# hkbharath/MARL-MASS

Hardware: AMD Instinct MI355X
Metric: agent-steps/sec (whole node), MASS CBF shield on, 65536 envs x 8 CAVs (higher is better)
Workload: dtype f64

## Files before the change

### include/mm_math.h

```cpp
#ifndef MM_MATH_H
#define MM_MATH_H

#ifndef MMM_FN
#define MMM_FN static inline
#endif

#if defined(__HIP_DEVICE_COMPILE__) && defined(__gfx950__)
MMM_FN double mmm_fma_c(double p, double z, double c) {
  double r;
  __asm__("v_fma_f64 %0, %1, %2, %3" : "=v"(r) : "v"(p), "v"(z), "s"(c));
  return r;
}
#else
#define mmm_fma_c(p, z, c) fma((p), (z), (c))
#endif

#define MMM_PIO2_1 0x1.921fb54400000p+0
#define MMM_PIO2_1T 0x1.0b4611a626331p-34
#define MMM_PIO2_HI 0x1.921fb54442d18p+0
#define MMM_PIO2_LO 0x1.1a62633145c07p-54
#define MMM_TWO_OVER_PI 0x1.45f306dc9c883p-1
#define MMM_LN2_HI 0x1.62e42ff000000p-1
#define MMM_LN2_LO -0x1.718432a1b0e26p-35
#define MMM_INV_LN2 0x1.71547652b82fep+0
// ... 136 lines not shown
  if (inv) r = MMM_PIO2_HI - (r - MMM_PIO2_LO);
  return x < 0 ? -r : r;
}
MMM_FN double mmm_atan_small(double x) {
  double t = fabs(x);
  double z = t * t;
  double p = MMM_K(mmm_t_atan, 0, MMM_A10);
  p = mmm_fma_c(p, z, MMM_K(mmm_t_atan, 1, MMM_A9)); p = mmm_fma_c(p, z, MMM_K(mmm_t_atan, 2, MMM_A8)); p = mmm_fma_c(p, z, MMM_K(mmm_t_atan, 3, MMM_A7)); p = mmm_fma_c(p, z, MMM_K(mmm_t_atan, 4, MMM_A6));
  p = mmm_fma_c(p, z, MMM_K(mmm_t_atan, 5, MMM_A5)); p = mmm_fma_c(p, z, MMM_K(mmm_t_atan, 6, MMM_A4)); p = mmm_fma_c(p, z, MMM_K(mmm_t_atan, 7, MMM_A3)); p = mmm_fma_c(p, z, MMM_K(mmm_t_atan, 8, MMM_A2));
  p = mmm_fma_c(p, z, MMM_K(mmm_t_atan, 9, MMM_A1));
  double r = fma(t * z, p, t);
  return x < 0 ? -r : r;
}
MMM_FN double mmm_asin_w(double x, double *w_out) {
  double y = fabs(x), lo;
  double w = sqrt((1.0 - y) * (1.0 + y));
  *w_out = w;
  const int direct = y <= w;
  double r = mmm_atan_ratio(direct ? y : w, direct ? w : y, &lo);
  if (!direct) r = MMM_PIO2_HI - (r - MMM_PIO2_LO);
  return x < 0 ? -r : r;
}
MMM_FN double mmm_asin(double x) { double w; return mmm_asin_w(x, &w); }
#define MMM_SIN_PI3 0x1.bb67ae8584caap-1
#define MMM_COS_PI3 0x1.0000000000001p-1
MMM_FN double mmm_exp(double x) {
  if (x < -1000.0) return 0.0;
  double k = rint(x * MMM_INV_LN2);
  double r = fma(-k, MMM_LN2_HI, x);
  r = fma(-k, MMM_LN2_LO, r);
  double p = MMM_K(mmm_t_exp, 0, MMM_E14);
  p = mmm_fma_c(p, r, MMM_K(mmm_t_exp, 1, MMM_E13)); p = mmm_fma_c(p, r, MMM_K(mmm_t_exp, 2, MMM_E12)); p = mmm_fma_c(p, r, MMM_K(mmm_t_exp, 3, MMM_E11)); p = mmm_fma_c(p, r, MMM_K(mmm_t_exp, 4, MMM_E10));
  p = mmm_fma_c(p, r, MMM_K(mmm_t_exp, 5, MMM_E9)); p = mmm_fma_c(p, r, MMM_K(mmm_t_exp, 6, MMM_E8)); p = mmm_fma_c(p, r, MMM_K(mmm_t_exp, 7, MMM_E7)); p = mmm_fma_c(p, r, MMM_K(mmm_t_exp, 8, MMM_E6));
  p = mmm_fma_c(p, r, MMM_K(mmm_t_exp, 9, MMM_E5)); p = mmm_fma_c(p, r, MMM_K(mmm_t_exp, 10, MMM_E4)); p = mmm_fma_c(p, r, MMM_K(mmm_t_exp, 11, MMM_E3)); p = mmm_fma_c(p, r, MMM_K(mmm_t_exp, 12, MMM_E2));
  p = fma(p, r * r, r) + 1.0;
  return ldexp(p, (int)k);
}
MMM_FN double mmm_log(double x) {
  int e;
  double m = frexp(x, &e);
  if (m < MMM_SQRT_HALF) { m = m * 2.0; e -= 1; }
  double f = m - 1.0;
  double s = f / (2.0 + f);
  double z = s * s;
  double p = MMM_K(mmm_t_log, 0, MMM_L11);
  p = mmm_fma_c(p, z, MMM_K(mmm_t_log, 1, MMM_L10)); p = mmm_fma_c(p, z, MMM_K(mmm_t_log, 2, MMM_L9)); p = mmm_fma_c(p, z, MMM_K(mmm_t_log, 3, MMM_L8)); p = mmm_fma_c(p, z, MMM_K(mmm_t_log, 4, MMM_L7));
// ... 19 lines not shown
```

### marl-mass_amd/csrc/mm_device.h

```cpp
#pragma once
#include <hip/hip_runtime.h>
#include <stdint.h>

#include "../../include/mm_abi.h"

#define MM_DEV __device__ __forceinline__
#define MMM_FN __device__ __forceinline__
#include "../../include/mm_math.h"
#ifndef MM_QP_NO_CERTIFY
#define MM_QP_CERTIFY
#endif
#include "../../include/mm_qp.h"

namespace mm {

constexpr double kPi = 3.141592653589793;
constexpr double kVehLength = 5.0, kVehWidth = 2.0, kMaxSpeed = 40.0;
constexpr double kTauA = 0.6, kTauDs = 0.2;
constexpr double kLcMaxAcc = 6.0, kLcMinAcc = -12.5;
constexpr double kPerception = 180.0, kStoppingSpeed = 1.6667;
constexpr double kLaneWidth = 4.0;
constexpr double kCbfAccLo = -12.5, kCbfAccHi = 6.0, kAdjBuffer = 2.0134;
constexpr double kSineAmp = 3.25, kSinePuls = 2 * kPi / (2 * 100.0), kSinePhase = kPi / 2;
constexpr double kObstX = 420.0, kObstY = 4.0;
constexpr double kT180 = 0x1.fa3ffffffffffp+14;
constexpr double kU5 = 0x1.9000000000001p+4;
constexpr double kCornerLen = 2.7000824035672517;
constexpr double kCornerAlpha = 0.3805063771123649;

MM_DEV double lane_sx(int l) { return l == 0 ? 0.0 : (l <= 2 ? 320.0 : (l == 3 ? 420.0 : (l == 4 ? 0.0 : 220.0))); }
MM_DEV double lane_sy(int l) { return l == 2 ? 4.0 : (l == 4 ? 10.5 : (l == 5 ? 7.25 : 0.0)); }
MM_DEV double lane_len(int l) { return l == 0 ? 320.0 : (l == 3 ? 1000.0 : (l == 4 ? 220.0 : 100.0)); }
MM_DEV bool lane_forbidden(int l) { return l == 2 || l >= 4; }
MM_DEV int lane_road(int l) { return l == 0 ? 0 : (l <= 2 ? 1 : l - 1); }
MM_DEV int lane_rid(int l) { return l == MM_LANE_BC1 ? 1 : 0; }

MM_DEV double fmod_pos(double a, double b) {
// ... 13 lines not shown
  if (m != 0.0) {
    if (m < 0) m += b;
  } else {
    m = 0.0;
  }
  return m;
}
MM_DEV double wrap_to_pi(double x) {
  const double a = x + kPi;
  if (__all(a >= 0.0 && a < 2 * kPi)) return a - kPi;
  return py_mod(a, 2 * kPi) - kPi;
}
MM_DEV double not_zero(double x) {
  return fabs(x) > 1e-2 ? x : (x > 0 ? 1e-2 : -1e-2);
}
MM_DEV double clipd(double x, double a, double b) { return fmin(fmax(x, a), b); }
MM_DEV double div_c(double x, double d, double y) {
  const double q = x * y;
  const double r = fma(-q, d, x);
  return fma(r, y, q);
}
#define MM_DIVC(x, d) ::mm::div_c((x), (d), 1.0 / (d))

MM_DEV void lane_local(int l, double x, double y, double &s, double &r) {
  s = x - lane_sx(l);
  r = y - lane_sy(l);
  if (l == MM_LANE_KB0) r = r - kSineAmp * mmm_sin(kSinePuls * s + kSinePhase);
}
MM_DEV void lane_local_carried(int l, double x, double y, double car, double &s, double &r) {
  s = x - lane_sx(l);
  r = y - lane_sy(l);
  const bool kb = l == MM_LANE_KB0;
  double sn = car;
  if (__any(kb && car != car)) sn = (car != car) ? mmm_sin(kSinePuls * s + kSinePhase) : car;
  if (kb) r = r - kSineAmp * sn;
}
static_assert(kSineAmp * kSinePuls * (1.0 + 0x1p-40) < 0.125, "the sine lane's heading needs the general mmm_atan");
template <bool SINE = false>
MM_DEV double lane_heading_at(int l, double s) {
  if constexpr (SINE) return l == MM_LANE_KB0 ? 0.0 + mmm_atan_small(kSineAmp * kSinePuls * mmm_cos(kSinePuls * s + kSinePhase)) : 0.0;
  else return l == MM_LANE_KB0 ? 0.0 + mmm_atan(kSineAmp * kSinePuls * mmm_cos(kSinePuls * s + kSinePhase)) : 0.0;
}
MM_DEV double lane_distance(int l, double x, double y) {
  double s, r;
  lane_local(l, x, y, s, r);
  return fabs(r) + fmax(s - lane_len(l), 0.0) + fmax(0.0 - s, 0.0);
}
MM_DEV bool lane_on_lane(int l, double x, double y) {
  double s, r;
  lane_local(l, x, y, s, r);
  return fabs(r) <= kLaneWidth / 2 + 0 && (-kVehLength <= s && s < lane_len(l) + kVehLength);
}
MM_DEV bool lane_reachable(int l, double x, double y) {
  if (lane_forbidden(l)) return false;
  double s = x - lane_sx(l), r = y - lane_sy(l);
  return fabs(r) <= 2 * kLaneWidth && (0 <= s && s < lane_len(l) + kVehLength);
}
MM_DEV bool lane_after_end(int l, double x) {
  return (x - lane_sx(l)) > lane_len(l) - kVehLength / 2;
}

template <bool SINE = false>
MM_DEV int closest_lane(double x, double y, double h, double *sine_out = nullptr) {
// ... 25 lines not shown
      double d = fabs(r) + tail + head + 1.0 * fabs(wrap_to_pi(h - lh));
      if (d < bd) { bd = d; best = MM_LANE_KB0; }
    }
  }
  return best;
}
MM_DEV int next_lane(int l, double x, double y) {
  if (l == MM_LANE_AB0 || l == MM_LANE_KB0)
    return lane_distance(MM_LANE_BC0, x, y) <= lane_distance(MM_LANE_BC1, x, y) ? MM_LANE_BC0 : MM_LANE_BC1;
  if (l == MM_LANE_JK0) return MM_LANE_KB0;
  return MM_LANE_CD0;
}

MM_DEV int speed_to_index(double speed) {
  double x = MM_DIVC(speed - 10, 20.0);
  return (int)clipd(rint(x * (5 - 1)), 0, 5 - 1);
}
MM_DEV double index_to_speed(int i) { return 10 + i * (30.0 - 10) / (5 - 1); }

template <bool SINE = false, bool CARRIED = false>
MM_DEV double steering_control(double x, double y, double heading, double speed, int tl, double &half_tan, double car = 0.0) {
  constexpr double KP_HEADING = 1 / kTauDs, KP_LATERAL = 1.0 / 3 * KP_HEADING, PURSUIT_TAU = 0.5 * kTauDs;
  double s, r;
  if constexpr (CARRIED) lane_local_carried(tl, x, y, car, s, r);
  else lane_local(tl, x, y, s, r);
  double lane_next = s + speed * PURSUIT_TAU;
  double lfh = lane_heading_at<SINE>(tl, lane_next);
  double lat_cmd = -KP_LATERAL * r;
  double nz = not_zero(speed);
  double heading_command = mmm_asin(clipd(lat_cmd / nz, -1, 1));
  double heading_ref = lfh + clipd(heading_command, -kPi / 4, kPi / 4);
  double rate = KP_HEADING * wrap_to_pi(heading_ref - heading);
  const double arg = clipd(kVehLength / 2 / nz * rate, -1, 1);
  double w;
  const double steer = mmm_asin_w(arg, &w);
  const bool sat = fabs(steer) > kPi / 3;
  const double ss = sat ? (arg < 0 ? -MMM_SIN_PI3 : MMM_SIN_PI3) : arg;
  const double cs = sat ? MMM_COS_PI3 : w;
  half_tan = 1.0 / 2 * (ss / cs);
  return clipd(steer, -kPi / 3, kPi / 3);
}
MM_DEV double steering_control(double x, double y, double heading, double speed, int tl) {
  double ht;
  return steering_control(x, y, heading, speed, tl, ht);
}

MM_DEV bool has_corner_inside(double c1x, double c1y, double l1, double w1, double a1, double c2x,
                              double c2y, double l2, double w2, double a2) {
  const double lx = l1 / 2, wy = w1 / 2;
  double c = mmm_cos(a1), s = mmm_sin(a1), c2 = mmm_cos(a2), s2 = mmm_sin(a2);
  const double px[9] = {0, -lx, lx, 0, 0, -lx, -lx, lx, lx};
  const double py[9] = {0, 0, 0, -wy, wy, -wy, wy, -wy, wy};
  bool any = false;
#pragma unroll
  for (int k = 0; k < 9; k++) {
    double rx = c * px[k] + (-s) * py[k], ry = s * px[k] + c * py[k];
    double dx = (c1x + rx) - c2x, dy = (c1y + ry) - c2y;
    double ru0 = c2 * dx + (-s2) * dy, ru1 = s2 * dx + c2 * dy;
// ... 37 lines not shown
```

### marl-mass_amd/csrc/mm_kernels.hip

```cpp
#include <hip/hip_runtime.h>
#include <math.h>
#include <stdio.h>
#include <string.h>

#include <type_traits>

#include "mm_device.h"
#include "mm_div.h"
#include "mm_handle.h"
#define MM_COUNTS_FN __host__ __device__ inline
#include "../../include/mm_counts.h"
#include "../../include/mm_policy_wide.h"

using namespace mm;

struct DevCfg {
  int env_kind, shield, nsub, T, action_masking, auto_reset, obs_f64, N, E, debug_flags, n_hdv;
  double dt, collision_reward, high_speed_reward, headway_cost, headway_time, merging_lane_cost;
  double rs_lo, rs_hi, eta, tau;
  double inv_dt, rs_span, rs_ispan, rs_span2, rs_ispan2;
  int agent_reward;
  int steer_vel;
  int *err;
  int traffic_density, mixed_traffic, num_cav;
// ... 60 lines not shown
    unsigned long long _t = __builtin_amdgcn_s_memtime();                                \
    if ((threadIdx.x & 63) == (k)) _t_acc += _t - _t_last;                               \
    _t_last = __builtin_amdgcn_s_memtime();                                              \
  } while (0)
enum { MM_CS_UPFRONT_CYCLES = 16,
       MM_CS_UPFRONT,
       MM_CS_LAZY_B,
       MM_CS_FALLBACK,
       MM_CS_PRIOR_HELD,
       MM_CS_PRIOR_LIFTED,
       MM_CS_LAZY_A,
       MM_CS_FIRST_B,
       MM_CS_NEAR,
       MM_CS_NEAR_ANY,
       MM_CS_PRECHECK,
       MM_CS_ROUND_CYCLES,
       MM_CS_ROUNDS,
       MM_CS_PASSES,
       MM_CS_SEED_ACTIVE,
       MM_CS_DIAG_CYCLES };
static_assert(MM_CS_DIAG_CYCLES == 31, "sixteen slots: lanes 16 .. 31");
constexpr bool mm_cs_is_cycles(int slot) { return slot == MM_CS_UPFRONT_CYCLES || slot == MM_CS_ROUND_CYCLES || slot == MM_CS_DIAG_CYCLES; }
__device__ unsigned long long g_stamps_c[MM_STAMP_WAVES * 16];
#define CAND_COUNT(k, cond)                                                                                  \
  do {                                                                                                       \
    const unsigned long long _m = __ballot(cond);                                                            \
    if ((threadIdx.x & 63) == (k)) _t_acc += (unsigned long long)__popcll(_m) + (_m ? 1ull << 32 : 0ull);    \
  } while (0)
#else
#define STAMP(k) do {} while (0)
#define SSTAMP(k) do {} while (0)
#define SCOUNT(k) do {} while (0)
#define CAND_COUNT(k, cond) do {} while (0)
#endif

template <int KIND> constexpr bool kIdm = KIND == MM_ENV_HDV_V1;

struct Veh {
  double x, y, h, v, tspeed;
  double act_steer, act_acc, safe_steer, safe_acc, gvx;
  double h1x, h1vx, h2x, h2vx;
  double sang;
  int lane, tlane, sidx, crashed, hl, flags, hist_len;
  int kind;
  bool present;
};
// ... 30 lines not shown
template <int M, int G, class F>
MM_DEV void for_partners_impl(F &f) {
  if constexpr (M < G) {
    f(std::integral_constant<int, M>{});
    for_partners_impl<M + 1, G>(f);
  }
}
template <int G, class F>
MM_DEV void for_partners(F f) { for_partners_impl<1, G>(f); }

template <int G> constexpr bool kPow2 = (G & (G - 1)) == 0;
#ifndef MM_ROUNDS_LITE
#define MM_ROUNDS_LITE 1
#endif
constexpr bool kRoundsLite = MM_ROUNDS_LITE != 0;
#ifndef MM_ROUNDS_PRIOR
#define MM_ROUNDS_PRIOR 1
#endif
constexpr bool kRoundsPrior = MM_ROUNDS_PRIOR != 0;
#ifndef MM_SCAN_SELECTS
#define MM_SCAN_SELECTS 1
#endif
constexpr bool kScanSelects = MM_SCAN_SELECTS != 0;
#ifndef MM_VETO_PRIOR
#define MM_VETO_PRIOR 1
#endif
constexpr bool kVetoPrior = MM_VETO_PRIOR != 0;
template <int M, int G>
MM_DEV int pidx(int a) {
  if constexpr (kPow2<G>) return a ^ M;
  else return a + M >= G ? a + M - G : a + M;
}
template <int G>
MM_DEV int pidx_rt(int a, int m) {
  if constexpr (kPow2<G>) return a ^ m;
  else return a + m >= G ? a + m - G : a + m;
}
template <int M, int G>
MM_DEV int plane(int lane, int a) {
  if constexpr (kPow2<G>) return lane ^ M;
  else return lane - a + pidx<M, G>(a);
}
template <int G>
MM_DEV int plane_rt(int lane, int a, int m) {
  if constexpr (kPow2<G>) return lane ^ m;
  else return lane - a + pidx_rt<G>(a, m);
// ... 90 lines not shown
    int cand = v.tlane;
    if (lane_road(v.tlane) == 1) cand = (action == 2) ? MM_LANE_BC1 : MM_LANE_BC0;
    if (lane_reachable(cand, v.x, v.y)) v.tlane = cand;
  }
  v.act_acc = (1 / kTauA) * (v.tspeed - v.v);
  if constexpr (STEER) steer_lane<SINE>(v, sv, st_t);
}
template <int KIND>
MM_DEV void hl_act(Veh &v, int action) {
  if (KIND == MM_ENV_V1 && action >= 0) v.hl = action;
  if (action == 3 || action == 4) {
    int si = speed_to_index(v.v) + (action == 3 ? 1 : -1);
    v.sidx = si < 0 ? 0 : (si > 4 ? 4 : si);
    v.tspeed = index_to_speed(v.sidx);
  }
  if (lane_after_end(v.tlane, v.x)) v.tlane = next_lane(v.tlane, v.x, v.y);
  if (action == 2 || action == 0) {
    int cand = v.tlane;
    if (lane_road(v.tlane) == 1) cand = (action == 2) ? MM_LANE_BC1 : MM_LANE_BC0;
    if (lane_reachable(cand, v.x, v.y)) v.tlane = cand;
  }
}

MM_DEV void clip_actions(Veh &v, bool lc_vehicle, double &st_t) {
  if (v.crashed) { v.act_steer = 0; st_t = 0; v.act_acc = -1.0 * v.v; }
  if (v.v > kMaxSpeed) v.act_acc = fmin(v.act_acc, 1.0 * (kMaxSpeed - v.v));
  else if (v.v < -kMaxSpeed) v.act_acc = fmax(v.act_acc, 1.0 * (kMaxSpeed - v.v));
  if (lc_vehicle) v.act_acc = clipd(v.act_acc, kLcMinAcc, kLcMaxAcc);
}

MM_DEV int corner_flags(double x, double y, double sh, double ch, int lane) {
  double cx = x + (kCornerLen * mmm_cos_sum(MMM_CORNER_SIN, MMM_CORNER_COS, sh, ch));
  double cyL = y - (kCornerLen * mmm_sin_sum(MMM_CORNER_SIN, MMM_CORNER_COS, sh, ch)) + 0.01;
  double cyR = y - (kCornerLen * mmm_sin_sum(-MMM_CORNER_SIN, MMM_CORNER_COS, sh, ch)) + 0.01;
  double s = cx - lane_sx(lane);
  double off = (lane == MM_LANE_KB0) ? kSineAmp * mmm_sin(kSinePuls * s + kSinePhase) : 0.0;
  bool lon = (-kVehLength <= s && s < lane_len(lane) + kVehLength);
  double rL = cyL - lane_sy(lane), rR = cyR - lane_sy(lane);
  if (lane == MM_LANE_KB0) { rL = rL - off; rR = rR - off; }
  return (!(fabs(rL) <= kLaneWidth / 2 + 0 && lon) ? 1 : 0) | (!(fabs(rR) <= kLaneWidth / 2 + 0 && lon) ? 2 : 0);
}
MM_DEV int pose_code(int lane, int nl, int off) { return lane | nl << 3 | off << 6; }

struct Cand {
  double x, y, h, gvx, cpsi, spsi;
  int lane;
  int pk;
};
template <int KIND, bool SHIELDED, bool CORNERS = SHIELDED, bool GENERAL = true, bool SINE = false>
MM_DEV Cand predict(const Veh &v, double steer, double st_t, double sh, double ch, double dt, bool sv = false, double *sine_out = nullptr) {
  Cand c;
  double ht = st_t, sb, cb;
  if constexpr (GENERAL) {
    if (__any(sv || st_t != st_t)) {
      double s2, c2;
      mmm_sincos(sv ? v.sang : steer, &s2, &c2);
      if (sv || st_t != st_t) ht = 1.0 / 2 * (s2 / c2);
    }
  }
  mmm_slip_sincos(ht, &sb, &cb);
  double vx = v.v * mmm_cos_sum(sh, ch, sb, cb), vy = v.v * mmm_sin_sum(sh, ch, sb, cb);
  c.x = v.x + vx * dt;
  c.y = v.y + vy * dt;
  const double d_heading = MM_DIVC(v.v * sb, 2.5);
  c.h = v.h + (sv ? d_heading : d_heading * dt);
  mmm_sincos(c.h, &c.spsi, &c.cpsi);
  c.gvx = (KIND == MM_ENV_V1) ? mmm_cos_sum(c.spsi, c.cpsi, sb, cb) : 0.0;
  c.lane = closest_lane<SINE>(c.x, c.y, c.h, sine_out);
  c.pk = c.lane;
  if (SHIELDED) c.pk = pose_code(c.lane, next_lane(c.lane, c.x, c.y), CORNERS ? corner_flags(c.x, c.y, c.spsi, c.cpsi, c.lane) : 0);
  return c;
}

MM_DEV int adj_pair(int l1, int l2) {
  return (l1 == MM_LANE_BC0 && l2 == MM_LANE_BC1) ? -1 : ((l1 == MM_LANE_BC1 && l2 == MM_LANE_BC0) ? 1 : 0);
}
MM_DEV int adj_lane(int l1, int nl1, int l2) {
  const int f = adj_pair(l1, l2);
  return f != 0 ? f : adj_pair(nl1, l2);
}
MM_DEV unsigned adj_row(int l1) { return l1 == MM_LANE_BC0 ? (3u << (2 * MM_LANE_BC1)) : (l1 == MM_LANE_BC1 ? (1u << (2 * MM_LANE_BC0)) : 0u); }
MM_DEV unsigned adj_col(int l2) { return l2 == MM_LANE_BC1 ? (3u << (2 * MM_LANE_BC0)) : (l2 == MM_LANE_BC0 ? (1u << (2 * MM_LANE_BC1)) : 0u); }

struct QpTrace {
  double rows, a, h0, h1, h2, h3, d, margin;
};

MM_DEV void init_vehicle(Veh &v) {
  v.lane = closest_lane(v.x, v.y, v.h);
  v.tlane = v.lane;
  v.act_steer = v.act_acc = 0;
  v.safe_steer = v.safe_acc = 0;
  if (v.kind == 2) {
// ... 884 lines not shown
#ifdef MM_SERIAL_ALL
  constexpr bool kSerialOnly = true || IPM;
#else
#ifdef MM_SERIAL_MASS
  constexpr bool kSerialOnly = MIXED || MASS || IPM;
#else
  constexpr bool kSerialOnly = MIXED;
#endif
#endif
  constexpr bool kSine = SHIELDED && !SPLIT && !MIXED && !IPM && !kSerialOnly && kPow2<G> && G <= 8;
  constexpr bool kScan = kScanSelects && !MIXED && !TRACE;
#ifndef MM_CARRY_POSE
#define MM_CARRY_POSE 1
#endif
  constexpr bool kCarry = kSine && MM_CARRY_POSE != 0;
#ifndef MM_PRIMARY_PRIOR
#define MM_PRIMARY_PRIOR 1
#endif
  constexpr bool kPrimary = kSine && !TRACE && kVetoPrior && MM_PRIMARY_PRIOR != 0;
#ifndef MM_SINE_CARRY
#define MM_SINE_CARRY 0
#endif
  constexpr bool kSineCarry = kPrimary && MM_SINE_CARRY != 0;
  double car_sn = __builtin_nan("");
  (void)car_sn;
  static_assert(kPow2<G> || MM_STEP_BLOCK == 64, "rotation layouts: one wave per workgroup");
  const long long gtid = (long long)blockIdx.x * blockDim.x + threadIdx.x;
  constexpr int kTail = kPow2<G> ? 64 : (64 / G) * G;
  const bool tail = lane_id() >= kTail;
  const int gb = kPow2<G> ? (lane_id() & ~(G - 1)) : (tail ? kTail - G : lane_id() - lane_id() % G);
  const int a = kPow2<G> ? (int)(gtid % G) : lane_id() - gb;
  const long long e = kPow2<G> ? gtid / G : (tail ? (long long)st.E : (gtid >> 6) * (64 / G) + lane_id() / G);
  const bool valid = e < st.E && a < st.N;
  const long long i = e * st.N + a;
  const long long A = st.A;
  const double dt = c.dt;

#ifdef MM_STAMPS
  unsigned long long _t_last = __builtin_amdgcn_s_memtime(), _t_acc = 0;
#endif
  Veh v;
  const bool sv = MIXED && KIND == MM_ENV_V1 && c.steer_vel != 0;
  int steps = 0, time = 0, n_merge = 0, episode = 0;
  int car_code = 0;
  long long car_kx = 0, car_ky = 0, car_kh = 0;
  double car_s = 0.0, car_c = 1.0;
  if constexpr (kCarry) {
    if (valid) {
      car_kx = __double_as_longlong(pb.F[PB_KX * A + i]); car_ky = __double_as_longlong(pb.F[PB_KY * A + i]);
      car_kh = __double_as_longlong(pb.F[PB_KH * A + i]);
      car_s = pb.F[PB_SIN * A + i]; car_c = pb.F[PB_COS * A + i]; car_code = pb.code[i];
    }
  }
  load_veh(st, i, valid, v, sv);
  if (e < st.E) {
    steps = st.I[MM_E_STEPS * st.E + e]; time = st.I[MM_E_TIME * st.E + e];
  }
  if (!MIXED && v.kind == 2) v.kind = 1;
  if (IDM && v.present) v.kind = 2;
  const bool hdv = MIXED && v.kind == 2;
  const bool ctrl = IDM ? v.present : (v.present && !hdv);
  const bool ctrl_x = IDM ? false : ctrl;
  int action = (!IDM && valid && ctrl) ? actions[i] : 1;
  if ((unsigned)action > 4u) {
    if (!SPLIT || kb == 0) atomicOr(c.err, MM_LATCH_BAD_ACTION);
    action = 1;
  }
  const unsigned present_bits = group_ballot<G>(v.present, gb);
  const unsigned ctrl_bits = group_ballot<G>(ctrl, gb);
  const int n_veh = __popc(present_bits), n_ctrl = __popc(ctrl_bits);
  if (!SPLIT || kb == 0) steps += 1;

  double cpsi = 1.0, spsi = 0.0;
  double st_t = __builtin_nan("");
  int pk_self = v.lane;
  bool carried = false;
  if constexpr (kCarry) {
    const bool hit = car_kx == __double_as_longlong(v.x) && car_ky == __double_as_longlong(v.y) && car_kh == __double_as_longlong(v.h) &&
                     (car_code >> 8) == ((kPoseWritten >> 8) | (MASS ? 1 : 0)) && (car_code & 7) == v.lane;
    carried = !__any(v.present && !hit);
    if (carried && v.present) { spsi = car_s; cpsi = car_c; pk_self = car_code & 0xFF; }
  }
  if (!carried) {
    if (v.present) mmm_sincos(v.h, &spsi, &cpsi);
    if (SHIELDED && v.present) pk_self = pose_code(v.lane, next_lane(v.lane, v.x, v.y), MASS ? corner_flags(v.x, v.y, spsi, cpsi, v.lane) : 0);
  }

  enum { C_B = 0, C_H1X = 8, C_H1VX, C_H2X, C_H2VX, C_SSTEER, C_SACC, C_TSPEED, C_A = 15, C_GU0 = 23, C_GU1 = 24, C_PRE = 25, C_MSGW = 29 };
  constexpr bool kMailbox = G <= 8 || !kPow2<G>;
  constexpr bool kPackMsg = !kPow2<G>;
  constexpr int kColdB = kMailbox ? (kPackMsg ? 29 : 30) : 25;
  constexpr bool kRoomy = false;
  constexpr int C_CPSI = kColdB + G - 1, C_GVX = C_CPSI + 1;
  constexpr int kColdN = !SHIELDED ? 15 : (kSerialOnly ? 23 : kColdB + G - 1 + (kRoomy ? 2 : 0));
  static_assert(kColdN * MM_STEP_BLOCK * 8 >= (MM_STEP_BLOCK / 64) * 64 * 30 * 4, "the obs staging must fit in the cold slots");
  __shared__ double s_cold[kColdN][MM_STEP_BLOCK];
  const int tid = threadIdx.x;
  auto cold_i = [&](int slot, int col) -> int & { return ((int *)&s_cold[slot][col])[0]; };
  if (LC) {
    s_cold[C_H1X][tid] = v.h1x; s_cold[C_H1VX][tid] = v.h1vx; s_cold[C_H2X][tid] = v.h2x; s_cold[C_H2VX][tid] = v.h2vx;
    s_cold[C_SSTEER][tid] = v.safe_steer; s_cold[C_SACC][tid] = v.safe_acc;
  }
  s_cold[C_TSPEED][tid] = v.tspeed;
  if constexpr (kRoomy) { s_cold[C_CPSI][tid] = cpsi; s_cold[C_GVX][tid] = v.gvx; }
  auto CPSI = [&]() -> double { if constexpr (kRoomy) return s_cold[C_CPSI][tid]; else return cpsi; };
  auto GVX = [&]() -> double { if constexpr (kRoomy) return s_cold[C_GVX][tid]; else return v.gvx; };
  bool env_active = IDM ? n_veh > 0 : n_ctrl > 0;
  if constexpr (SPLIT) {
    if (kb > 0) env_active = e < st.E && sb.envf[e] != 0;
  }
  STAMP(0);
  const int k_lo = SPLIT ? (kb > 0 ? kb - 1 : 0) : 0, k_hi = SPLIT ? (kb < c.nsub ? kb : c.nsub - 1) : c.nsub - 1;
  for (int k = k_lo; k <= k_hi; k++) {
    const bool head = !SPLIT || k == kb, tail = !SPLIT || k != kb;
    const bool live = env_active && v.present;
    QpTrace qt = {0, __builtin_nan(""), __builtin_nan(""), __builtin_nan(""), __builtin_nan(""),
                  __builtin_nan(""), __builtin_nan(""), __builtin_nan("")};
    int rank = 0;
    if ((SHIELDED || MIXED) && head) {
      for_partners<G>([&](auto mc) {
        constexpr int m = decltype(mc)::value;
        double px = px_d<m, G>(v.x, a);
        bool pp = px_i<m, G>((int)live, a) != 0;
        if constexpr (kScan) rank += (pp & ((px > v.x) | ((px == v.x) & (pidx<m, G>(a) < a)))) ? 1 : 0;
        else rank += (pp && (px > v.x || (px == v.x && pidx<m, G>(a) < a))) ? 1 : 0;
      });
// ... 88 lines not shown
          const int nxt = (acting && lc_branch) ? ((same_road && hit) ? v.lane : my_tl) : tl_post;
          const bool changed = nxt != tl_post;
          tl_post = nxt;
          if (!__any(changed)) break;
        }
        if constexpr (MIXED) { STAMP(5); }
        if (acting) {
          v.tlane = tl_post;
          v.act_acc = clipd(acc_f0, -6.0, 6.0);
        }
      }
      if (head && live && (!hdv || !v.crashed)) steer_lane(v, sv && !hdv, st_t);
      if (head && hdv && live) v.gvx += dt;
    }
    bool first_B = false;
    if constexpr (kPrimary) {
      static_assert(!MIXED && !SPLIT, "kPrimary: no HDVs, no steer_vel, every launch a whole step");
      first_B = (c.debug_flags & 1) == 0 && live && v.hist_len >= 2 && (v.tlane != v.lane || v.crashed) && !(v.flags & MM_FLAG_IS_LC_SAFE);
      if (live) {
        const int tl_1 = v.tlane + (first_B ? v.lane - v.tlane : 0);
        const double steer = steering_control<kSine, kSineCarry>(v.x, v.y, v.h, v.v, tl_1, st_t, car_sn);
        v.act_steer = clipd(steer, -kPi / 3, kPi / 3);
        const double steer_1 = v.act_steer, st_t_1 = st_t;
        clip_actions(v, LC, st_t);
        if (first_B) { v.act_steer = steer_1; st_t = st_t_1; }
      }
    } else {
      if (live && head) clip_actions(v, LC && !hdv, st_t);
    }
    STAMP(1);
    Cand cA;
    memset(&cA, 0, sizeof cA);
    const bool shield_on = SHIELDED && live && !hdv && v.hist_len >= 2;
    if constexpr (kSineCarry) car_sn = __builtin_nan("");
    if (live && head) cA = predict<KIND, SHIELDED, MASS, MIXED, kSine>(v, v.act_steer, st_t, spsi, cpsi, dt, sv && !hdv, kSineCarry ? &car_sn : nullptr);
    auto park = [&](auto base_c, const Cand &cc, double steer) {
      constexpr int base = decltype(base_c)::value;
      if constexpr (SHIELDED) {
        s_cold[base + 0][tid] = cc.x; s_cold[base + 1][tid] = cc.y; s_cold[base + 2][tid] = cc.h;
        cold_i(base + 3, tid) = cc.pk; s_cold[base + 4][tid] = cc.cpsi; s_cold[base + 5][tid] = steer;
        s_cold[base + 6][tid] = cc.gvx; s_cold[base + 7][tid] = cc.spsi;
      }
    };
    auto park_at = [&](int base, const Cand &cc, double steer) {
      s_cold[base + 0][tid] = cc.x; s_cold[base + 1][tid] = cc.y; s_cold[base + 2][tid] = cc.h;
      cold_i(base + 3, tid) = cc.pk; s_cold[base + 4][tid] = cc.cpsi; s_cold[base + 5][tid] = steer;
      s_cold[base + 6][tid] = cc.gvx; s_cold[base + 7][tid] = cc.spsi;
    };
    if constexpr (kPrimary) park_at(first_B ? (int)C_B : (int)C_A, cA, v.act_steer);
    else if (head) park(std::integral_constant<int, C_A>{}, cA, v.act_steer);
    STAMP(2);
// ... 712 lines not shown
    if (is_mdp(i_rr)) { sum += r_rr; cnt++; }
    regional = sum / cnt;
  }
  double rsum = 0, ssum = 0, tsum = 0;
#pragma unroll
  for (int q = 0; q < G; q++) {
    const double lr = shfl_d(local, gb + q), sp = shfl_d(v.v, gb + q);
    const bool in = q < st.N, cq = in & (((ctrl_bits >> q) & 1u) != 0), pq = in & (((present_bits >> q) & 1u) != 0);
    const double r1 = rsum + lr, s1 = ssum + sp, t1 = tsum + sp;
    rsum = cq ? r1 : rsum; ssum = cq ? s1 : ssum;
    tsum = pq ? t1 : tsum;
  }
  const double reward = env_ok ? rsum / n_ctrl : 0, avg_speed = env_ok ? ssum / n_ctrl : 0;
  const double traffic_speed = env_ok ? tsum / n_veh : 0;
  double th = INFINITY;
  if (ctrl) {
    double h2d = hd;
    if (fabs(kObstY - v.y) <= 2 && kObstX > v.x) { double dd = kObstX - v.x; if (dd < h2d) h2d = dd; }
    h2d = h2d - kVehLength;
    double vx = v.v * cpsi;
    th = h2d / (vx > 1 ? vx : 1);
  }
  const double min_headway = group_min_d<G>(th, a);
  if (e < st.E) { n_merge = st.I[MM_E_N_MERGE * st.E + e]; episode = st.I[MM_E_EPISODE * st.E + e]; }
  double merge_pct = __builtin_nan("");
  if (done) {
    const int n_rem = __popc(group_ballot<G>(
        ctrl && (v.lane == MM_LANE_BC1 || v.lane == MM_LANE_KB0 || v.lane == MM_LANE_JK0), gb));
    merge_pct = n_merge > 0 ? (double)(n_merge - n_rem) / n_merge * 100 : 100.0;
  }
  if (valid) {
    if (out.agents_rewards) out.agents_rewards[i] = ctrl ? local : 0;
    if (out.regional_rewards) out.regional_rewards[i] = ctrl ? regional : 0;
    if (out.agents_dones) out.agents_dones[i] = ctrl ? (uint8_t)(v.crashed || steps >= c.T || v.x < 0) : 1;
    if (out.crashed) out.crashed[i] = v.present ? (uint8_t)v.crashed : 0;
    if (out.agents_info) {
      out.agents_info[i * 3 + 0] = v.present ? v.x : 0;
      out.agents_info[i * 3 + 1] = v.present ? v.y : 0;
      out.agents_info[i * 3 + 2] = v.present ? v.v : 0;
    }
  }
  if (e < st.E && a == 0 && env_ok) {
    if (out.reward) out.reward[e] = reward;
    if (out.done) out.done[e] = (uint8_t)done;
    if (out.average_speed) out.average_speed[e] = avg_speed;
    if (out.traffic_speed) out.traffic_speed[e] = traffic_speed;
    if (out.min_headway) out.min_headway[e] = min_headway;
// ... 39 lines not shown
    memset(&nv, 0, sizeof nv);
    int nm = 0;
    int nc = n_ctrl, nh = n_veh - n_ctrl;
    if constexpr (IDM) { nc = 0; nh = n_veh; }
    episode_counts<KIND>(c, seed, (uint32_t)episode, nc, nh);
    const bool spawn = valid && (c.traffic_density > 0 ? a < nc + nh : v.present);
    if (spawn) nm = spawn_vehicle(nv, a, nc, nh, seed, (uint32_t)episode);
    if (c.traffic_density > 0 && valid) {
      if (!spawn) {
        if (v.present) {
          Veh z;
          memset(&z, 0, sizeof z);
          store_veh(st, i, z, true);
        }
        v.present = false; v.kind = 0;
      }
      st.B[MM_B_KIND * A + i] = spawn ? (uint8_t)nv.kind : (uint8_t)0;
    }
    if (spawn) {
      v = nv;
      spsi = 0.0; cpsi = 1.0;
      if constexpr (kCarry) {
        mmm_sincos(v.h, &car_s, &car_c);
        pk_self = pose_code(v.lane, next_lane(v.lane, v.x, v.y), MASS ? corner_flags(v.x, v.y, car_s, car_c, v.lane) : 0);
      }
      s_cold[C_H1X][tid] = v.h1x; s_cold[C_H1VX][tid] = v.h1vx; s_cold[C_H2X][tid] = v.h2x; s_cold[C_H2VX][tid] = v.h2vx;
      s_cold[C_SSTEER][tid] = v.safe_steer; s_cold[C_SACC][tid] = v.safe_acc; s_cold[C_TSPEED][tid] = v.tspeed;
    }
    n_merge = shfl_i(nm, gb);
    steps = 0; time = 0; episode += 1;
  }
  if (valid && v.present) {
    if (LC) {
      v.h1x = s_cold[C_H1X][tid]; v.h1vx = s_cold[C_H1VX][tid]; v.h2x = s_cold[C_H2X][tid]; v.h2vx = s_cold[C_H2VX][tid];
      if (!hdv) { v.safe_steer = s_cold[C_SSTEER][tid]; v.safe_acc = s_cold[C_SACC][tid]; }
    }
    v.tspeed = s_cold[C_TSPEED][tid];
    store_veh(st, i, v, sv);
    if constexpr (kCarry) {
      pb.F[PB_KX * A + i] = v.x; pb.F[PB_KY * A + i] = v.y; pb.F[PB_KH * A + i] = v.h;
      pb.F[PB_SIN * A + i] = car_s; pb.F[PB_COS * A + i] = car_c;
      pb.code[i] = (pk_self & 0xFF) | (MASS ? 0x100 : 0) | kPoseWritten;
    }
  }
  if (e < st.E && a == 0) {
    st.I[MM_E_STEPS * st.E + e] = steps; st.I[MM_E_TIME * st.E + e] = time;
    st.I[MM_E_N_MERGE * st.E + e] = n_merge; st.I[MM_E_EPISODE * st.E + e] = episode;
  }
  STAMP(11);
  __syncthreads();
  STAMP(14);
  const double sc_h[2] = {spsi, cpsi};
  observe<G, KIND, true, kScan>(c, v, a, gb, i, valid, out.obs, out.action_mask, (float *)&s_cold[0][0], sc_h);
  STAMP(12);
#ifdef MM_STAMPS
  {
    const long long wv = gtid >> 6;
    if ((threadIdx.x & 63) < 16 && wv < MM_STAMP_WAVES) g_stamps_w[wv * 16 + (threadIdx.x & 63)] += _t_acc;
    else if ((threadIdx.x & 63) < 32 && wv < MM_STAMP_WAVES) g_stamps_c[wv * 16 + (threadIdx.x & 63) - 16] += _t_acc;
  }
#endif
}

template <int G, int KIND>
__global__ __launch_bounds__(256) void reset_kernel(DevCfg c, DevState st, int mode, const uint8_t *env_mask,
                                                    const uint64_t *seeds_in, void *obs, uint8_t *avail) {
  const long long gtid = (long long)blockIdx.x * blockDim.x + threadIdx.x;
  const long long e = gtid / G;
  const int a = (int)(gtid % G);
  const int gb = lane_id() & ~(G - 1);
  const bool valid = e < st.E && a < st.N;
  const long long i = e * st.N + a;
  const bool selected = e < st.E && mode != 2 && (!env_mask || env_mask[e]);
  Veh v;
  load_veh(st, i, valid, v);
  if (kIdm<KIND> && v.present) v.kind = 2;
  if (selected) {
    int steps = 0, time = 0, n_merge = 0, episode = st.I[MM_E_EPISODE * st.E + e];
    if (mode == 0) {
      if (seeds_in && a == 0) st.seeds[e] = seeds_in[e];
      const uint64_t seed = seeds_in ? seeds_in[e] : st.seeds[e];
      int nm = 0;
// ... 1125 lines not shown
  hipError_t rc = hipMemcpyFromSymbol(host, HIP_SYMBOL(g_stamps_s), sizeof host);
  for (int k = 0; k < 8; k++) out8[k] = 0;
  for (int w = 0; w < 4096; w++)
    for (int k = 0; k < 8; k++) out8[k] += host[w * 8 + k];
  if (rc == hipSuccess && reset) {
    memset(host, 0, sizeof host);
    rc = hipMemcpyToSymbol(HIP_SYMBOL(g_stamps_s), host, sizeof host);
  }
  return rc == hipSuccess ? MM_OK : MM_ERR_DEVICE;
}
extern "C" int32_t mm_debug_read_stamps(unsigned long long *out16, int32_t reset) {
  static unsigned long long *host = nullptr;
  if (!host) host = (unsigned long long *)malloc(sizeof(unsigned long long) * MM_STAMP_WAVES * 16);
  hipError_t rc = hipMemcpyFromSymbol(host, HIP_SYMBOL(g_stamps_w), sizeof(unsigned long long) * MM_STAMP_WAVES * 16);
  for (int k = 0; k < 16; k++) out16[k] = 0;
  for (long long w = 0; w < MM_STAMP_WAVES; w++)
    for (int k = 0; k < 16; k++) out16[k] += host[w * 16 + k];
  if (rc == hipSuccess && reset) {
    memset(host, 0, sizeof(unsigned long long) * MM_STAMP_WAVES * 16);
    rc = hipMemcpyToSymbol(HIP_SYMBOL(g_stamps_w), host, sizeof(unsigned long long) * MM_STAMP_WAVES * 16);
  }
  return rc == hipSuccess ? MM_OK : MM_ERR_DEVICE;
}
extern "C" int32_t mm_debug_read_cand_stamps(unsigned long long *out32, int32_t reset) {
  static unsigned long long *host = nullptr;
  if (!host) host = (unsigned long long *)malloc(sizeof(unsigned long long) * MM_STAMP_WAVES * 16);
  hipError_t rc = hipMemcpyFromSymbol(host, HIP_SYMBOL(g_stamps_c), sizeof(unsigned long long) * MM_STAMP_WAVES * 16);
  for (int k = 0; k < 32; k++) out32[k] = 0;
  for (long long w = 0; w < MM_STAMP_WAVES; w++)
    for (int k = 0; k < 16; k++) {
      const unsigned long long x = host[w * 16 + k];
      if (mm_cs_is_cycles(k + 16)) { out32[k] += x; continue; }
      out32[k] += x & 0xFFFFFFFFull;
      out32[16 + k] += x >> 32;
    }
  if (rc == hipSuccess && reset) {
    memset(host, 0, sizeof(unsigned long long) * MM_STAMP_WAVES * 16);
    rc = hipMemcpyToSymbol(HIP_SYMBOL(g_stamps_c), host, sizeof(unsigned long long) * MM_STAMP_WAVES * 16);
  }
  return rc == hipSuccess ? MM_OK : MM_ERR_DEVICE;
}
#endif
#endif
```

Baseline: 2.534 billion.

## Use branch-free select variants for trig, asin, corner flags and action clipping; hoist loads

Adds select-based sin/cos, atan-ratio and asin variants that compute both kernels and pick the result instead of branching. It also makes corner_flags and clip_actions branch-free on the sine path, and moves the action and per-env episode counter loads to the top of the step kernel. The counters are stashed in the free high words of shared slots. The goal is less wave divergence and earlier memory latency, paid for with extra ALU work per lane and some shared-memory aliasing. Per-wave timing records are added under the stamps debug build only.

After: 2.595 billion (median of 6 runs). +2.4%, better.

```diff
diff --git a/include/mm_math.h b/include/mm_math.h
--- a/include/mm_math.h
+++ b/include/mm_math.h
@@ -182,6 +182,49 @@
   return x < 0 ? -r : r;
 }
 MMM_FN double mmm_asin(double x) { double w; return mmm_asin_w(x, &w); }
+
+MMM_FN double mmm_sin_sel(double x) {
+  int q;
+  double r = mmm_reduce(x, &q);
+  double ks = mmm_ksin(r), kc = mmm_kcos(r);
+  double s = (q & 1) ? kc : ks;
+  return (q & 2) ? -s : s;
+}
+MMM_FN double mmm_cos_sel(double x) {
+  int q;
+  double r = mmm_reduce(x, &q);
+  double ks = mmm_ksin(r), kc = mmm_kcos(r);
+  double c = (q & 1) ? ks : kc;
+  return ((q + 1) & 2) ? -c : c;
+}
+MMM_FN double mmm_atan_ratio_sel(double num, double den, double *lo_out) {
+  const int j = (num >= 0.125 * den) + (num >= 0.375 * den) + (num >= 0.625 * den) + (num >= 0.875 * den);
+  double c = 0.25 * (double)j;
+  double t = (num - c * den) / (den + c * num);
+  double z = t * t;
+  double p = MMM_K(mmm_t_atan, 0, MMM_A10);
+  p = mmm_fma_c(p, z, MMM_K(mmm_t_atan, 1, MMM_A9)); p = mmm_fma_c(p, z, MMM_K(mmm_t_atan, 2, MMM_A8)); p = mmm_fma_c(p, z, MMM_K(mmm_t_atan, 3, MMM_A7)); p = mmm_fma_c(p, z, MMM_K(mmm_t_atan, 4, MMM_A6));
+  p = mmm_fma_c(p, z, MMM_K(mmm_t_atan, 5, MMM_A5)); p = mmm_fma_c(p, z, MMM_K(mmm_t_atan, 6, MMM_A4)); p = mmm_fma_c(p, z, MMM_K(mmm_t_atan, 7, MMM_A3)); p = mmm_fma_c(p, z, MMM_K(mmm_t_atan, 8, MMM_A2));
+  p = mmm_fma_c(p, z, MMM_K(mmm_t_atan, 9, MMM_A1));
+  double pt = fma(t * z, p, t);
+  double hi = 0.0, lo = 0.0;
+  hi = j >= 1 ? MMM_ATAN_HI_1 : hi; lo = j >= 1 ? MMM_ATAN_LO_1 : lo;
+  hi = j >= 2 ? MMM_ATAN_HI_2 : hi; lo = j >= 2 ? MMM_ATAN_LO_2 : lo;
+  hi = j >= 3 ? MMM_ATAN_HI_3 : hi; lo = j >= 3 ? MMM_ATAN_LO_3 : lo;
+  hi = j >= 4 ? MMM_ATAN_HI_4 : hi; lo = j >= 4 ? MMM_ATAN_LO_4 : lo;
+  *lo_out = lo;
+  return hi + (pt + lo);
+}
+MMM_FN double mmm_asin_w_sel(double x, double *w_out) {
+  double y = fabs(x), lo;
+  double w = sqrt((1.0 - y) * (1.0 + y));
+  *w_out = w;
+  const int direct = y <= w;
+  double r = mmm_atan_ratio_sel(direct ? y : w, direct ? w : y, &lo);
+  if (!direct) r = MMM_PIO2_HI - (r - MMM_PIO2_LO);
+  return x < 0 ? -r : r;
+}
+MMM_FN double mmm_asin_sel(double x) { double w; return mmm_asin_w_sel(x, &w); }
 #define MMM_SIN_PI3 0x1.bb67ae8584caap-1
 #define MMM_COS_PI3 0x1.0000000000001p-1
 MMM_FN double mmm_exp(double x) {
diff --git a/marl-mass_amd/csrc/mm_device.h b/marl-mass_amd/csrc/mm_device.h
--- a/marl-mass_amd/csrc/mm_device.h
+++ b/marl-mass_amd/csrc/mm_device.h
@@ -13,6 +13,25 @@
 #include "../../include/mm_qp.h"
 
 namespace mm {
+
+#ifndef MM_TRIG_SELECTS
+#define MM_TRIG_SELECTS 1
+#endif
+#ifndef MM_ATAN_SELECTS
+#define MM_ATAN_SELECTS 1
+#endif
+#ifndef MM_CORNER_SELECTS
+#define MM_CORNER_SELECTS 1
+#endif
+#ifndef MM_CLIP_SELECTS
+#define MM_CLIP_SELECTS 1
+#endif
+constexpr bool kTrigSelects = MM_TRIG_SELECTS != 0, kAtanSelects = MM_ATAN_SELECTS != 0;
+constexpr bool kCornerSelects = MM_CORNER_SELECTS != 0, kClipSelects = MM_CLIP_SELECTS != 0;
+template <bool SEL> MM_DEV double sin_f(double x) { if constexpr (SEL && kTrigSelects) return mmm_sin_sel(x); else return mmm_sin(x); }
+template <bool SEL> MM_DEV double cos_f(double x) { if constexpr (SEL && kTrigSelects) return mmm_cos_sel(x); else return mmm_cos(x); }
+template <bool SEL> MM_DEV double asin_f(double x) { if constexpr (SEL && kAtanSelects) return mmm_asin_sel(x); else return mmm_asin(x); }
+template <bool SEL> MM_DEV double asin_w_f(double x, double *w) { if constexpr (SEL && kAtanSelects) return mmm_asin_w_sel(x, w); else return mmm_asin_w(x, w); }
 
 constexpr double kPi = 3.141592653589793;
 constexpr double kVehLength = 5.0, kVehWidth = 2.0, kMaxSpeed = 40.0;
@@ -72,23 +91,25 @@
 }
 #define MM_DIVC(x, d) ::mm::div_c((x), (d), 1.0 / (d))
 
+template <bool SEL = false>
 MM_DEV void lane_local(int l, double x, double y, double &s, double &r) {
   s = x - lane_sx(l);
   r = y - lane_sy(l);
-  if (l == MM_LANE_KB0) r = r - kSineAmp * mmm_sin(kSinePuls * s + kSinePhase);
-}
+  if (l == MM_LANE_KB0) r = r - kSineAmp * sin_f<SEL>(kSinePuls * s + kSinePhase);
+}
+template <bool SEL = false>
 MM_DEV void lane_local_carried(int l, double x, double y, double car, double &s, double &r) {
   s = x - lane_sx(l);
   r = y - lane_sy(l);
   const bool kb = l == MM_LANE_KB0;
   double sn = car;
-  if (__any(kb && car != car)) sn = (car != car) ? mmm_sin(kSinePuls * s + kSinePhase) : car;
+  if (__any(kb && car != car)) sn = (car != car) ? sin_f<SEL>(kSinePuls * s + kSinePhase) : car;
   if (kb) r = r - kSineAmp * sn;
 }
 static_assert(kSineAmp * kSinePuls * (1.0 + 0x1p-40) < 0.125, "the sine lane's heading needs the general mmm_atan");
 template <bool SINE = false>
 MM_DEV double lane_heading_at(int l, double s) {
-  if constexpr (SINE) return l == MM_LANE_KB0 ? 0.0 + mmm_atan_small(kSineAmp * kSinePuls * mmm_cos(kSinePuls * s + kSinePhase)) : 0.0;
+  if constexpr (SINE) return l == MM_LANE_KB0 ? 0.0 + mmm_atan_small(kSineAmp * kSinePuls * cos_f<true>(kSinePuls * s + kSinePhase)) : 0.0;
   else return l == MM_LANE_KB0 ? 0.0 + mmm_atan(kSineAmp * kSinePuls * mmm_cos(kSinePuls * s + kSinePhase)) : 0.0;
 }
 MM_DEV double lane_distance(int l, double x, double y) {
@@ -160,18 +181,18 @@
 MM_DEV double steering_control(double x, double y, double heading, double speed, int tl, double &half_tan, double car = 0.0) {
   constexpr double KP_HEADING = 1 / kTauDs, KP_LATERAL = 1.0 / 3 * KP_HEADING, PURSUIT_TAU = 0.5 * kTauDs;
   double s, r;
-  if constexpr (CARRIED) lane_local_carried(tl, x, y, car, s, r);
-  else lane_local(tl, x, y, s, r);
+  if constexpr (CARRIED) lane_local_carried<SINE>(tl, x, y, car, s, r);
+  else lane_local<SINE>(tl, x, y, s, r);
   double lane_next = s + speed * PURSUIT_TAU;
   double lfh = lane_heading_at<SINE>(tl, lane_next);
   double lat_cmd = -KP_LATERAL * r;
   double nz = not_zero(speed);
-  double heading_command = mmm_asin(clipd(lat_cmd / nz, -1, 1));
+  double heading_command = asin_f<SINE>(clipd(lat_cmd / nz, -1, 1));
   double heading_ref = lfh + clipd(heading_command, -kPi / 4, kPi / 4);
   double rate = KP_HEADING * wrap_to_pi(heading_ref - heading);
   const double arg = clipd(kVehLength / 2 / nz * rate, -1, 1);
   double w;
-  const double steer = mmm_asin_w(arg, &w);
+  const double steer = asin_w_f<SINE>(arg, &w);
   const bool sat = fabs(steer) > kPi / 3;
   const double ss = sat ? (arg < 0 ? -MMM_SIN_PI3 : MMM_SIN_PI3) : arg;
   const double cs = sat ? MMM_COS_PI3 : w;
diff --git a/marl-mass_amd/csrc/mm_kernels.hip b/marl-mass_amd/csrc/mm_kernels.hip
--- a/marl-mass_amd/csrc/mm_kernels.hip
+++ b/marl-mass_amd/csrc/mm_kernels.hip
@@ -106,6 +106,9 @@
 static_assert(MM_CS_DIAG_CYCLES == 31, "sixteen slots: lanes 16 .. 31");
 constexpr bool mm_cs_is_cycles(int slot) { return slot == MM_CS_UPFRONT_CYCLES || slot == MM_CS_ROUND_CYCLES || slot == MM_CS_DIAG_CYCLES; }
 __device__ unsigned long long g_stamps_c[MM_STAMP_WAVES * 16];
+#define MM_REC_WAVES (1 << 14)
+enum { MM_REC_BEGIN, MM_REC_END, MM_REC_RT_BEGIN, MM_REC_RT_END, MM_REC_HW, MM_REC_RESPAWN, MM_REC_SLOTS = 8, MM_REC_WORDS = 40 };
+__device__ unsigned long long g_wave_rec[MM_REC_WAVES * MM_REC_WORDS];
 #define CAND_COUNT(k, cond)                                                                                  \
   do {                                                                                                       \
     const unsigned long long _m = __ballot(cond);                                                            \
@@ -182,6 +185,9 @@
 #define MM_SCAN_SELECTS 1
 #endif
 constexpr bool kScanSelects = MM_SCAN_SELECTS != 0;
+#ifndef MM_EARLY_LOADS
+#define MM_EARLY_LOADS 1
+#endif
 #ifndef MM_VETO_PRIOR
 #define MM_VETO_PRIOR 1
 #endif
@@ -318,19 +324,43 @@
   }
 }
 
+template <bool SEL = false>
 MM_DEV void clip_actions(Veh &v, bool lc_vehicle, double &st_t) {
+  if constexpr (SEL && kClipSelects) {
+    const bool cr = v.crashed != 0;
+    v.act_steer = cr ? 0.0 : v.act_steer; st_t = cr ? 0.0 : st_t;
+    double acc = cr ? -1.0 * v.v : v.act_acc;
+    const double room = 1.0 * (kMaxSpeed - v.v);
+    const bool over = v.v > kMaxSpeed, under = !over & (v.v < -kMaxSpeed);
+    const double a_lo = fmin(acc, room), a_hi = fmax(acc, room);
+    acc = over ? a_lo : (under ? a_hi : acc);
+    const double a_lc = clipd(acc, kLcMinAcc, kLcMaxAcc);
+    v.act_acc = lc_vehicle ? a_lc : acc;
+  } else {
   if (v.crashed) { v.act_steer = 0; st_t = 0; v.act_acc = -1.0 * v.v; }
   if (v.v > kMaxSpeed) v.act_acc = fmin(v.act_acc, 1.0 * (kMaxSpeed - v.v));
   else if (v.v < -kMaxSpeed) v.act_acc = fmax(v.act_acc, 1.0 * (kMaxSpeed - v.v));
   if (lc_vehicle) v.act_acc = clipd(v.act_acc, kLcMinAcc, kLcMaxAcc);
-}
-
+  }
+}
+
+template <bool SEL = false>
 MM_DEV int corner_flags(double x, double y, double sh, double ch, int lane) {
   double cx = x + (kCornerLen * mmm_cos_sum(MMM_CORNER_SIN, MMM_CORNER_COS, sh, ch));
   double cyL = y - (kCornerLen * mmm_sin_sum(MMM_CORNER_SIN, MMM_CORNER_COS, sh, ch)) + 0.01;
   double cyR = y - (kCornerLen * mmm_sin_sum(-MMM_CORNER_SIN, MMM_CORNER_COS, sh, ch)) + 0.01;
   double s = cx - lane_sx(lane);
-  double off = (lane == MM_LANE_KB0) ? kSineAmp * mmm_sin(kSinePuls * s + kSinePhase) : 0.0;
+  if constexpr (SEL && kCornerSelects) {
+    const bool kb = lane == MM_LANE_KB0;
+    double sn = 0.0;
+    if (kb) sn = sin_f<true>(kSinePuls * s + kSinePhase);
+    const double off = kb ? kSineAmp * sn : 0.0;
+    const bool lon = (-kVehLength <= s) & (s < lane_len(lane) + kVehLength);
+    const double rL0 = cyL - lane_sy(lane), rR0 = cyR - lane_sy(lane);
+    const double rL = kb ? rL0 - off : rL0, rR = kb ? rR0 - off : rR0;
+    return (!((fabs(rL) <= kLaneWidth / 2 + 0) & lon) ? 1 : 0) | (!((fabs(rR) <= kLaneWidth / 2 + 0) & lon) ? 2 : 0);
+  }
+  double off = (lane == MM_LANE_KB0) ? kSineAmp * sin_f<SEL>(kSinePuls * s + kSinePhase) : 0.0;
   bool lon = (-kVehLength <= s && s < lane_len(lane) + kVehLength);
   double rL = cyL - lane_sy(lane), rR = cyR - lane_sy(lane);
   if (lane == MM_LANE_KB0) { rL = rL - off; rR = rR - off; }
@@ -364,7 +394,7 @@
   c.gvx = (KIND == MM_ENV_V1) ? mmm_cos_sum(c.spsi, c.cpsi, sb, cb) : 0.0;
   c.lane = closest_lane<SINE>(c.x, c.y, c.h, sine_out);
   c.pk = c.lane;
-  if (SHIELDED) c.pk = pose_code(c.lane, next_lane(c.lane, c.x, c.y), CORNERS ? corner_flags(c.x, c.y, c.spsi, c.cpsi, c.lane) : 0);
+  if (SHIELDED) c.pk = pose_code(c.lane, next_lane(c.lane, c.x, c.y), CORNERS ? corner_flags<SINE>(c.x, c.y, c.spsi, c.cpsi, c.lane) : 0);
   return c;
 }
 
@@ -1295,6 +1325,7 @@
 #define MM_SINE_CARRY 0
 #endif
   constexpr bool kSineCarry = kPrimary && MM_SINE_CARRY != 0;
+  constexpr bool kEarly = kSine && MM_EARLY_LOADS != 0;
   double car_sn = __builtin_nan("");
   (void)car_sn;
   static_assert(kPow2<G> || MM_STEP_BLOCK == 64, "rotation layouts: one wave per workgroup");
@@ -1310,6 +1341,7 @@
   const double dt = c.dt;
 
 #ifdef MM_STAMPS
+  const unsigned long long _rec_t0 = __builtin_amdgcn_s_memtime(), _rec_rt0 = __builtin_amdgcn_s_memrealtime();
   unsigned long long _t_last = __builtin_amdgcn_s_memtime(), _t_acc = 0;
 #endif
   Veh v;
@@ -1318,6 +1350,12 @@
   int car_code = 0;
   long long car_kx = 0, car_ky = 0, car_kh = 0;
   double car_s = 0.0, car_c = 1.0;
+  int act_raw = 1;
+  (void)act_raw;
+  if constexpr (kEarly) {
+    if (valid) act_raw = actions[i];
+    if (e < st.E) { n_merge = st.I[MM_E_N_MERGE * st.E + e]; episode = st.I[MM_E_EPISODE * st.E + e]; }
+  }
   if constexpr (kCarry) {
     if (valid) {
       car_kx = __double_as_longlong(pb.F[PB_KX * A + i]); car_ky = __double_as_longlong(pb.F[PB_KY * A + i]);
@@ -1334,7 +1372,9 @@
   const bool hdv = MIXED && v.kind == 2;
   const bool ctrl = IDM ? v.present : (v.present && !hdv);
   const bool ctrl_x = IDM ? false : ctrl;
-  int action = (!IDM && valid && ctrl) ? actions[i] : 1;
+  int action;
+  if constexpr (kEarly) action = ctrl ? act_raw : 1;
+  else action = (!IDM && valid && ctrl) ? actions[i] : 1;
   if ((unsigned)action > 4u) {
     if (!SPLIT || kb == 0) atomicOr(c.err, MM_LATCH_BAD_ACTION);
     action = 1;
@@ -1356,7 +1396,7 @@
   }
   if (!carried) {
     if (v.present) mmm_sincos(v.h, &spsi, &cpsi);
-    if (SHIELDED && v.present) pk_self = pose_code(v.lane, next_lane(v.lane, v.x, v.y), MASS ? corner_flags(v.x, v.y, spsi, cpsi, v.lane) : 0);
+    if (SHIELDED && v.present) pk_self = pose_code(v.lane, next_lane(v.lane, v.x, v.y), MASS ? corner_flags<kSine>(v.x, v.y, spsi, cpsi, v.lane) : 0);
   }
 
   enum { C_B = 0, C_H1X = 8, C_H1VX, C_H2X, C_H2VX, C_SSTEER, C_SACC, C_TSPEED, C_A = 15, C_GU0 = 23, C_GU1 = 24, C_PRE = 25, C_MSGW = 29 };
@@ -1375,6 +1415,10 @@
     s_cold[C_SSTEER][tid] = v.safe_steer; s_cold[C_SACC][tid] = v.safe_acc;
   }
   s_cold[C_TSPEED][tid] = v.tspeed;
+  if constexpr (kEarly) {
+    static_assert(kMailbox && !kPackMsg, "the high words of the pose-code and rank-word slots must be free");
+    ((int *)&s_cold[C_PRE + 3][tid])[1] = n_merge; ((int *)&s_cold[C_MSGW][tid])[1] = episode;
+  }
   if constexpr (kRoomy) { s_cold[C_CPSI][tid] = cpsi; s_cold[C_GVX][tid] = v.gvx; }
   auto CPSI = [&]() -> double { if constexpr (kRoomy) return s_cold[C_CPSI][tid]; else return cpsi; };
   auto GVX = [&]() -> double { if constexpr (kRoomy) return s_cold[C_GVX][tid]; else return v.gvx; };
@@ -1509,11 +1553,11 @@
         const double steer = steering_control<kSine, kSineCarry>(v.x, v.y, v.h, v.v, tl_1, st_t, car_sn);
         v.act_steer = clipd(steer, -kPi / 3, kPi / 3);
         const double steer_1 = v.act_steer, st_t_1 = st_t;
-        clip_actions(v, LC, st_t);
+        clip_actions<kSine>(v, LC, st_t);
         if (first_B) { v.act_steer = steer_1; st_t = st_t_1; }
       }
     } else {
-      if (live && head) clip_actions(v, LC && !hdv, st_t);
+      if (live && head) clip_actions<kSine>(v, LC && !hdv, st_t);
     }
     STAMP(1);
     Cand cA;
@@ -2272,7 +2316,8 @@
     th = h2d / (vx > 1 ? vx : 1);
   }
   const double min_headway = group_min_d<G>(th, a);
-  if (e < st.E) { n_merge = st.I[MM_E_N_MERGE * st.E + e]; episode = st.I[MM_E_EPISODE * st.E + e]; }
+  if constexpr (kEarly) { n_merge = ((const int *)&s_cold[C_PRE + 3][tid])[1]; episode = ((const int *)&s_cold[C_MSGW][tid])[1]; }
+  else if (e < st.E) { n_merge = st.I[MM_E_N_MERGE * st.E + e]; episode = st.I[MM_E_EPISODE * st.E + e]; }
   double merge_pct = __builtin_nan("");
   if (done) {
     const int n_rem = __popc(group_ballot<G>(
@@ -2358,7 +2403,7 @@
       spsi = 0.0; cpsi = 1.0;
       if constexpr (kCarry) {
         mmm_sincos(v.h, &car_s, &car_c);
-        pk_self = pose_code(v.lane, next_lane(v.lane, v.x, v.y), MASS ? corner_flags(v.x, v.y, car_s, car_c, v.lane) : 0);
+        pk_self = pose_code(v.lane, next_lane(v.lane, v.x, v.y), MASS ? corner_flags<kSine>(v.x, v.y, car_s, car_c, v.lane) : 0);
       }
       s_cold[C_H1X][tid] = v.h1x; s_cold[C_H1VX][tid] = v.h1vx; s_cold[C_H2X][tid] = v.h2x; s_cold[C_H2VX][tid] = v.h2vx;
       s_cold[C_SSTEER][tid] = v.safe_steer; s_cold[C_SACC][tid] = v.safe_acc; s_cold[C_TSPEED][tid] = v.tspeed;
@@ -2394,6 +2439,19 @@
     const long long wv = gtid >> 6;
     if ((threadIdx.x & 63) < 16 && wv < MM_STAMP_WAVES) g_stamps_w[wv * 16 + (threadIdx.x & 63)] += _t_acc;
     else if ((threadIdx.x & 63) < 32 && wv < MM_STAMP_WAVES) g_stamps_c[wv * 16 + (threadIdx.x & 63) - 16] += _t_acc;
+    if (wv < MM_REC_WAVES) {
+      unsigned long long *rec = g_wave_rec + wv * MM_REC_WORDS;
+      const int respawned = __popcll(__ballot(c.auto_reset && done && a == 0 && e < st.E));
+      if ((threadIdx.x & 63) < 32) rec[MM_REC_SLOTS + (threadIdx.x & 63)] = _t_acc;
+      if ((threadIdx.x & 63) == 0) {
+        const unsigned hw = __builtin_amdgcn_s_getreg(4 | (31 << 11)), xcc = __builtin_amdgcn_s_getreg(20 | (31 << 11));
+        rec[MM_REC_BEGIN] = _rec_t0; rec[MM_REC_RT_BEGIN] = _rec_rt0;
+        rec[MM_REC_HW] = (unsigned long long)hw | (unsigned long long)xcc << 32;
+        rec[MM_REC_RESPAWN] = (unsigned long long)respawned;
+        rec[MM_REC_RT_END] = __builtin_amdgcn_s_memrealtime();
+        rec[MM_REC_END] = __builtin_amdgcn_s_memtime();
+      }
+    }
   }
 #endif
 }
@@ -3565,6 +3623,11 @@
   }
   return rc == hipSuccess ? MM_OK : MM_ERR_DEVICE;
 }
+extern "C" int32_t mm_debug_read_wave_records(unsigned long long *out, int32_t n_waves) {
+  if (!out || n_waves <= 0 || n_waves > MM_REC_WAVES) return MM_ERR_INVALID_ARG;
+  hipError_t rc = hipMemcpyFromSymbol(out, HIP_SYMBOL(g_wave_rec), sizeof(unsigned long long) * MM_REC_WORDS * (size_t)n_waves);
+  return rc == hipSuccess ? MM_OK : MM_ERR_DEVICE;
+}
 extern "C" int32_t mm_debug_read_cand_stamps(unsigned long long *out32, int32_t reset) {
   static unsigned long long *host = nullptr;
   if (!host) host = (unsigned long long *)malloc(sizeof(unsigned long long) * MM_STAMP_WAVES * 16);
```
